# bgmanuel99/Super-Resolution-Images-for-3D-Printing-Defect-Detection

Measured on AMD Instinct MI355X. Metric: 4x-SR MPix/s on 512x512 LR batch, higher is better.
Workload: dtype bf16

## Files before the change

### super-resolution-images-for-3d-printing-defect-detection_amd/csrc/dense_fused.hip

```cpp
#include <stdlib.h>
#include <string.h>

#include <type_traits>

#include "conv_common.h"

namespace {

struct ChainParams {
    const char* in; int in_nch;
    char* out; int out_nch;
    const char* so; int so_nch;
    const char* w;
    const float* bias;
    const char* zero;
    int B, H;
    int rows_per_wg; unsigned magic;
    float alpha, xscale, oscale;
    int dbg_flags;
    unsigned long long* dbg;
};

__device__ __forceinline__ f32x4 mma16(bf16x8 a, bf16x8 b, f32x4 c) { return __builtin_amdgcn_mfma_f32_16x16x32_bf16(a, b, c, 0, 0, 0); }

constexpr int ROWB = 3072;
constexpr int NSTG = 11;
constexpr int STGB = NSTG * ROWB;
constexpr int WINR = 10;
constexpr int ZERO_PAGE_BYTES = sr_ctx::ZERO_PAGE_BYTES;

template <int NB0, int NB1, int MODE> struct ChainLds {
    static constexpr int WSLOT = (NB0 + NB1) * 3 * 1024;
    static constexpr int NSB = MODE == 0 ? 3 : 2;
    static constexpr int NWS = MODE == 0 ? 2 : 3;
    static constexpr int BYTES = NSB * STGB + WINR * ROWB + NWS * WSLOT + (NB0 + NB1) * 16 * 4;
};

typedef unsigned u32x2 __attribute__((ext_vector_type(2)));
typedef unsigned u32x4 __attribute__((ext_vector_type(4)));
#define CHAIN_STAMP(k) do { if (STAMP && blockIdx.x < 64 && G < 64 && (wave == 0 || wave == 5 || wave == 8 || wave == 11) && lane == 0)                \
        p.dbg[(((size_t)blockIdx.x * 4 + (wave == 0 ? 0 : wave == 5 ? 1 : wave == 8 ? 2 : 3)) * 64 + G) * 4 + (k)] = __builtin_amdgcn_s_memtime(); } while (0)

template <int N, class F> __device__ __forceinline__ void static_for(F&& f) {
    if constexpr (N > 0) {
        static_for<N - 1>(f);
        f(std::integral_constant<int, N - 1>{});
    }
}

template <int N> __device__ __forceinline__ void wait_imm() {
    static_assert(N >= 0 && N < 64, "vmcnt is a 6-bit counter");
    asm volatile("s_waitcnt vmcnt(%0)" ::"n"(N) : "memory");
}

template <int EXT, int NB0, int NB1, int MODE, int LW> struct LoaderPlan {
    static constexpr int NBT = NB0 + NB1, EXTG = 3 * EXT, NGR = 3 * (EXT + 1);
    static constexpr int RT_E = MODE == 1 ? 2 : 3;
    static constexpr int RT_R = 2;
    static constexpr int nrows(int kx) { return kx == 0 ? 2 : kx == 1 ? (LW < 3 ? 1 : 0) : 0; }
    static constexpr int nst_at(int i) {
        i = (i % NGR + NGR) % NGR;
        return i < EXTG ? 3 * nrows(i % 3) : 0;
    }
    static constexpr int nwdma(int iw) {
        const bool ext = iw < EXTG;
        const int nw = ext ? NBT * 3 : NB1 * 3, rt = ext ? RT_E : RT_R;
        int n = 0;
        for (int t = 0; t < (nw + 3) / 4; ++t)
            if (LW + 4 * t < nw && t >= rt) ++n;
        return n;
    }
};

constexpr bool kDirectStores = true;
constexpr int NCOMP = 8, NLOAD = 4;

template <int EXT, int NB0, int NB1, int MODE, bool HAS_O, bool STAMP, bool SEAM = false>
__global__ void __launch_bounds__((NCOMP + NLOAD) * 64, (NCOMP + NLOAD + 3) / 4) chain2_kernel(ChainParams p) {
    using L = ChainLds<NB0, NB1, MODE>;
    constexpr int NBT = NB0 + NB1, WSLOT = L::WSLOT;
    constexpr int NGR = 3 * (EXT + 1);
    constexpr int EXTG = 3 * EXT;
    constexpr int NTHR = (NCOMP + NLOAD) * 64;
    extern __shared__ __attribute__((aligned(16))) char smem[];
    char* const stg = smem;
    constexpr int NSB = L::NSB;
    char* const win = smem + NSB * STGB;
    char* const wr = win + WINR * ROWB;
    constexpr int NWS = L::NWS;
    float* const lbias = reinterpret_cast<float*>(wr + NWS * WSLOT);

    const int tid = threadIdx.x, lane = tid & 63, px = lane & 15, q = lane >> 4;
    const int wave = __builtin_amdgcn_readfirstlane(tid >> 6);
    const int H = p.H, Hp1 = H + 1;
    const int T = p.B * Hp1;
    const int R0 = blockIdx.x * p.rows_per_wg, R1 = min(T, R0 + p.rows_per_wg);
    if (R0 >= R1) return;
    const int Rs = R0 - 1;
    const int N = R1 - Rs + 1;
    const int nsteps = (N + 1 + 7) >> 3;

    for (int u = tid; u < WINR * ROWB / 16; u += NTHR) *reinterpret_cast<f32x4*>(win + u * 16) = f32x4{0.f, 0.f, 0.f, 0.f};
    if (tid < NBT * 16) lbias[tid] = p.bias[tid];
    asm volatile("s_waitcnt lgkmcnt(0)" ::: "memory");
    __builtin_amdgcn_s_barrier();

    auto row_of = [&](int g, int& img, int& y) -> bool {
        const int gg = Rs + g;
        if (gg < 0 || gg >= T) return false;
        img = (int)__umulhi((unsigned)gg, p.magic);
        y = gg - img * Hp1;
        return y < H;
    };
    auto own = [&](int g) { return Rs + g >= R0 && Rs + g < R1; };
    int G = 0;
    auto dma = [&](const char* src, char* dst) {
        __builtin_amdgcn_global_load_lds((const __attribute__((address_space(1))) void*)src, (__attribute__((address_space(3))) void*)dst, 16, 0, 0);
    };
    if (wave >= NCOMP) {
        const int lwr = wave - NCOMP;
        const int lsrc = 64 * (lane >> 2) + 16 * ((lane & 3) ^ (2 * ((lane >> 4) & 1)));
        auto loader = [&](auto LWc) {
            constexpr int LW = decltype(LWc)::value;
            auto row_base = [&](int s2, int j) -> const char* {
                int img, y;
                const bool real = row_of(8 * s2 - 2 + j, img, y);
                return real ? p.in + ((int64_t)img * H + y) * p.in_nch * ROWB : p.zero;
            };
            using Plan = LoaderPlan<EXT, NB0, NB1, MODE, LW>;
            const char* rb_cur[3];
            const char* rb_nxt[3];
            auto bases_of = [&](int s2, const char* (&rb)[3]) {
                rb[0] = row_base(s2, LW);
                rb[1] = row_base(s2, LW + 4);
                rb[2] = row_base(s2, 8 + (LW < 3 ? LW : 2));
            };
            auto stage_row = [&](auto Jc, const char* rb, int c1, char* sdst) {
                constexpr int j = decltype(Jc)::value;
                const char* src = rb + c1 * ROWB + lsrc;
                char* dst = sdst + j * ROWB;
                const auto gs = (const __attribute__((address_space(1))) void*)src;
                const auto ld = (__attribute__((address_space(3))) void*)dst;
                if constexpr (j < 8) {
                    __builtin_amdgcn_global_load_lds(gs, ld, 16, 0, 2);
                    __builtin_amdgcn_global_load_lds(gs, ld, 16, 1024, 2);
                    __builtin_amdgcn_global_load_lds(gs, ld, 16, 2048, 2);
                } else {
                    __builtin_amdgcn_global_load_lds(gs, ld, 16, 0, 0);
                    __builtin_amdgcn_global_load_lds(gs, ld, 16, 1024, 0);
                    __builtin_amdgcn_global_load_lds(gs, ld, 16, 2048, 0);
                }
            };
            auto stage_rows = [&](auto KXc, const char* (&rb)[3], int c1, char* sdst) {
                constexpr int kx = decltype(KXc)::value;
                if constexpr (kx == 0) {
                    stage_row(std::integral_constant<int, LW>{}, rb[0], c1, sdst);
                    stage_row(std::integral_constant<int, LW + 4>{}, rb[1], c1, sdst);
                } else if constexpr (kx == 1 && LW < 3) {
                    stage_row(std::integral_constant<int, 8 + (LW < 3 ? LW : 0)>{}, rb[2], c1, sdst);
                }
            };
            constexpr int RT_E = Plan::RT_E, RT_R = Plan::RT_R;
            u32x4 wre[EXTG][RT_E], wrr[3][RT_R];
            auto wsrc_of = [&](int iw) { return p.w + (iw < EXTG ? iw * WSLOT : EXTG * WSLOT + (iw - EXTG) * (NB1 * 3 * 1024)); };
#pragma unroll
            for (int iw = 0; iw < EXTG; ++iw)
#pragma unroll
                for (int t = 0; t < RT_E; ++t)
                    if (LW + 4 * t < NBT * 3) wre[iw][t] = *reinterpret_cast<const u32x4*>(wsrc_of(iw) + (LW + 4 * t) * 1024 + lane * 16);
#pragma unroll
            for (int r = 0; r < 3; ++r)
#pragma unroll
                for (int t = 0; t < RT_R; ++t)
                    if (LW + 4 * t < NB1 * 3) wrr[r][t] = *reinterpret_cast<const u32x4*>(wsrc_of(EXTG + r) + (LW + 4 * t) * 1024 + lane * 16);
            auto put_weights = [&](auto IW, int Gw) {
                constexpr int iw = decltype(IW)::value;
                constexpr bool ext = iw < EXTG;
                constexpr int nw = ext ? NBT * 3 : NB1 * 3, rt = ext ? RT_E : RT_R;
                const char* wq = p.w;
                asm volatile("" : "+s"(wq));
                const char* wsrc = wq + (ext ? iw * WSLOT : EXTG * WSLOT + (iw - EXTG) * (NB1 * 3 * 1024)) + lane * 16;
                char* wdst = wr + (Gw % NWS) * WSLOT;
#pragma unroll
                for (int t = 0; t < (nw + 3) / 4; ++t) {
                    const int k = LW + 4 * t;
                    if (k < nw) {
                        if (t < rt) {
                            if constexpr (ext) *reinterpret_cast<u32x4*>(wdst + k * 1024 + lane * 16) = wre[ext ? iw : 0][t < RT_E ? t : 0];
                            else *reinterpret_cast<u32x4*>(wdst + k * 1024 + lane * 16) = wrr[ext ? 0 : iw - EXTG][t < RT_R ? t : 0];
                        } else {
                            dma(wsrc + k * 1024, wdst + k * 1024);
                        }
                    }
                }
            };
            constexpr int WL = NWS - 1;
            constexpr int SL = NSB - 1;
            static_assert(MODE == 1 || (RT_E * NLOAD >= NBT * 3 && RT_R * NLOAD >= NB1 * 3), "growth pairs: every weight piece is resident (no weight DMA in the counted waits)");
            static_assert(SL <= EXT, "rows run at most one step ahead");
            static_for<WL>([&](auto I) { put_weights(I, decltype(I)::value); });
            bases_of(0, rb_cur);
            bases_of(1, rb_nxt);
            static_for<SL>([&](auto C0) {
                constexpr int c0 = decltype(C0)::value;
                stage_rows(std::integral_constant<int, 0>{}, rb_cur, c0, stg + c0 * STGB);
                stage_rows(std::integral_constant<int, 1>{}, rb_cur, c0, stg + c0 * STGB);
            });
            int nch = 0;
            for (int s = 0; s < nsteps; ++s) {
                static_for<NGR>([&](auto I) {
                    constexpr int i = decltype(I)::value;
                    CHAIN_STAMP(0);
                    if (G == 0) asm volatile("s_waitcnt vmcnt(0)" ::: "memory");
                    asm volatile("s_waitcnt lgkmcnt(0)" ::: "memory");
                    __builtin_amdgcn_s_barrier();
                    CHAIN_STAMP(1);
                    constexpr int i2 = (i + WL) % NGR;
                    put_weights(std::integral_constant<int, i2>{}, G + WL);
                    if constexpr (i < EXTG) {
                        constexpr int c = i / 3, kx = i - 3 * c;
                        constexpr int c1 = (c + SL) % EXT;
                        constexpr bool next_step = c + SL >= EXT;
                        char* sdst = stg + ((nch + SL) % NSB) * STGB;
                        stage_rows(std::integral_constant<int, kx>{}, next_step ? rb_nxt : rb_cur, c1, sdst);
                        if (kx == 2) ++nch;
                    }
                    CHAIN_STAMP(2);
                    if constexpr (MODE == 0) {
                        wait_imm<Plan::nst_at(i) + Plan::nst_at(i - 1) + Plan::nst_at(i - 2)>();
                    } else {
                        constexpr bool third = i < EXTG && i % 3 == 2;
                        wait_imm<Plan::nwdma(i2) + Plan::nst_at(i) + (third ? 0 : Plan::nst_at(i - 1))>();
                    }
                    CHAIN_STAMP(3);
                    ++G;
                });
                rb_cur[0] = rb_nxt[0]; rb_cur[1] = rb_nxt[1]; rb_cur[2] = rb_nxt[2];
                bases_of(s + 2, rb_nxt);
            }
            asm volatile("s_waitcnt vmcnt(0)" ::: "memory");
        };
        if (lwr == 0) loader(std::integral_constant<int, 0>{});
        else if (lwr == 1) loader(std::integral_constant<int, 1>{});
        else if (lwr == 2) loader(std::integral_constant<int, 2>{});
        else loader(std::integral_constant<int, 3>{});
        return;
    }

    int offk[3];
#pragma unroll
    for (int kx = 0; kx < 3; ++kx) {
        const int c = px + kx - 1;
        offk[kx] = 64 * c + 16 * (q ^ (2 * ((c >> 2) & 1)));
    }
    const bool edge_l = px == 0, edge_r = px == 15;
    const int off_l = edge_l ? offk[1] : offk[0];
    const int off_r = edge_r ? offk[1] : offk[2];
    const bool seam_l = SEAM && px == 8, seam_r = SEAM && px == 7;

    f32x4 a0[NB0][3], a1[NB1][3];

    auto transpose_offsets = [&](int& t_a, int& t_line) {
        int l = lane;
        asm volatile("" : "+v"(l));
        const int px_ = l & 15, q_ = l >> 4;
        t_a = px_ * 64 + 16 * ((q_ >> 1) ^ ((px_ >> 1) & 3)) + (q_ & 1) * 8;
        t_line = (l >> 2) * 64 + 16 * ((l & 3) ^ ((l >> 3) & 3));
    };

    auto xfold = [&](int h, float scale) {
        const bf16_t xs_b = (bf16_t)scale;
        int j0 = 16 * h + px - 8 * q;
        asm volatile("" : "+v"(j0));
        bf16x8 f;
#pragma unroll
        for (int j = 0; j < 8; ++j) f[j] = j == j0 ? xs_b : (bf16_t)0.f;
        return f;
    };
    constexpr int WDEPTH = 3, NWREG = WDEPTH + 1;
    struct ExtStage { int d, layer, n, frag, first; };
    auto ext_stage = [](int k) constexpr -> ExtStage {
        int i = 0;
        for (int d = 0; d < 4; ++d) {
            bool first = true;
            if (d >= 1)
                for (int n = 0; n < NB0; ++n, ++i, first = false)
                    if (i == k) return ExtStage{d, 0, n, (d - 1) * NB0 + n, first};
            if (d <= 2)
                for (int n = 0; n < NB1; ++n, ++i, first = false)
                    if (i == k) return ExtStage{d, 1, n, 3 * NB0 + d * NB1 + n, first};
        }
        return ExtStage{-1, 0, 0, 0, 0};
    };
    constexpr int NEXTST = 3 * (NB0 + NB1);
    auto ext_granule = [&](auto KXc, auto FOLDc, const char* sb, const char* ws) {
        constexpr int KX = decltype(KXc)::value;
        constexpr int FOLD = KX == 1 ? decltype(FOLDc)::value : -1;
        const char* rb = sb + wave * ROWB;
        auto load_row = [&](int d, bf16x8 (&x)[3]) {
#pragma unroll
            for (int cg = 0; cg < 3; ++cg) {
                const int off = (KX == 0 && cg == 0) ? off_l : (KX == 2 && cg == 2) ? off_r : offk[KX];
                x[cg] = *reinterpret_cast<const bf16x8*>(rb + d * ROWB + cg * 1024 + off);
                if ((KX == 0 && cg == 0 && edge_l) || (KX == 2 && cg == 2 && edge_r)) x[cg] = bf16x8{};
                if (SEAM && cg == 1 && ((KX == 0 && seam_l) || (KX == 2 && seam_r))) x[cg] = bf16x8{};
            }
        };
        auto ldw = [&](int frag) { return *reinterpret_cast<const bf16x8*>(ws + frag * 1024 + lane * 16); };
        bf16x8 xr[2][3], wq[NWREG];
        load_row(0, xr[0]);
        static_for<WDEPTH>([&](auto K) { wq[decltype(K)::value] = ldw(ext_stage(decltype(K)::value).frag); });
        static_for<NEXTST>([&](auto K) {
            constexpr int k = decltype(K)::value;
            constexpr ExtStage st = ext_stage(k);
            if constexpr (st.first && st.d < 3) load_row(st.d + 1, xr[(st.d + 1) & 1]);
            if constexpr (k + WDEPTH < NEXTST) wq[(k + WDEPTH) % NWREG] = ldw(ext_stage(k + WDEPTH).frag);
#pragma unroll
            for (int cg = 0; cg < 3; ++cg) {
                if constexpr (st.layer == 0) a0[st.n][cg] = mma16(wq[k % NWREG], xr[st.d & 1][cg], a0[st.n][cg]);
                else a1[st.n][cg] = mma16(wq[k % NWREG], xr[st.d & 1][cg], a1[st.n][cg]);
            }
            if constexpr (FOLD >= 0 && st.d == 1 && st.layer == 1 && st.n == NB1 - 1) {
#pragma unroll
                for (int h = 0; h < 2; ++h) {
                    const bf16x8 f = xfold(h, p.xscale);
#pragma unroll
                    for (int cg = 0; cg < 3; ++cg) a1[2 * FOLD + h][cg] = mma16(f, xr[1][cg], a1[2 * FOLD + h][cg]);
                }
            }
            __builtin_amdgcn_sched_barrier(0);
        });
    };
    constexpr int NRINGST = 3 * NB1;
    auto ring_granule = [&](auto KXc, int s, const char* ws) {
        constexpr int KX = decltype(KXc)::value;
        auto load_row = [&](int ky, bf16x8 (&x)[3]) {
            const char* rb = win + ((8 * s + wave - 2 + ky + 2 * WINR) % WINR) * ROWB;
#pragma unroll
            for (int cg = 0; cg < 3; ++cg) {
                const int off = (KX == 0 && cg == 0) ? off_l : (KX == 2 && cg == 2) ? off_r : offk[KX];
                x[cg] = *reinterpret_cast<const bf16x8*>(rb + cg * 1024 + off);
                if ((KX == 0 && cg == 0 && edge_l) || (KX == 2 && cg == 2 && edge_r)) x[cg] = bf16x8{};
                if (SEAM && cg == 1 && ((KX == 0 && seam_l) || (KX == 2 && seam_r))) x[cg] = bf16x8{};
            }
        };
        auto ldw = [&](int frag) { return *reinterpret_cast<const bf16x8*>(ws + frag * 1024 + lane * 16); };
        bf16x8 xr[2][3], wq[NWREG];
        load_row(0, xr[0]);
        static_for<WDEPTH>([&](auto K) { wq[decltype(K)::value] = ldw(decltype(K)::value); });
        static_for<NRINGST>([&](auto K) {
            constexpr int k = decltype(K)::value;
            constexpr int ky = k / NB1, n = k % NB1;
            if constexpr (n == 0 && ky < 2) load_row(ky + 1, xr[(ky + 1) & 1]);
            if constexpr (k + WDEPTH < NRINGST) wq[(k + WDEPTH) % NWREG] = ldw(k + WDEPTH);
#pragma unroll
            for (int cg = 0; cg < 3; ++cg) a1[n][cg] = mma16(wq[k % NWREG], xr[ky & 1][cg], a1[n][cg]);
            __builtin_amdgcn_sched_barrier(0);
        });
    };
    auto sync = [&]() {
        asm volatile("s_waitcnt lgkmcnt(0)" ::: "memory");
        __builtin_amdgcn_s_barrier();
    };

    int nch = 0;
    auto chunk = [&](auto FOLDc, int& Gr) {
        const char* sb = stg + (nch % NSB) * STGB;
#pragma unroll
        for (int kx = 0; kx < 3; ++kx, ++Gr) {
            CHAIN_STAMP(0);
            sync();
            CHAIN_STAMP(1);
            CHAIN_STAMP(2);
            const char* ws = wr + (Gr % NWS) * WSLOT;
            if (STAMP && (p.dbg_flags & 2)) {  }
            else if (kx == 0) ext_granule(std::integral_constant<int, 0>{}, FOLDc, sb, ws);
            else if (kx == 1) ext_granule(std::integral_constant<int, 1>{}, FOLDc, sb, ws);
            else ext_granule(std::integral_constant<int, 2>{}, FOLDc, sb, ws);
            CHAIN_STAMP(3);
        }
        ++nch;
    };
    for (int s = 0; s < nsteps; ++s) {
#pragma unroll
        for (int n = 0; n < NB0; ++n) {
            const f32x4 b = *reinterpret_cast<const f32x4*>(lbias + n * 16 + 4 * q);
#pragma unroll
            for (int cg = 0; cg < 3; ++cg) a0[n][cg] = b;
        }
#pragma unroll
        for (int n = 0; n < NB1; ++n) {
            const f32x4 b = *reinterpret_cast<const f32x4*>(lbias + (NB0 + n) * 16 + 4 * q);
#pragma unroll
            for (int cg = 0; cg < 3; ++cg) a1[n][cg] = b;
        }
        if constexpr (MODE == 1) {
            static_assert(MODE == 0 || EXT >= 2, "the tail's skip spans chunks 0 and 1");
            chunk(std::integral_constant<int, 0>{}, G);
            chunk(std::integral_constant<int, 1>{}, G);
#pragma nounroll
            for (int c = 2; c < EXT; ++c) chunk(std::integral_constant<int, -1>{}, G);
        } else {
#pragma nounroll
            for (int c = 0; c < EXT; ++c) chunk(std::integral_constant<int, -1>{}, G);
        }
        {
            const int g0 = 8 * s + wave;
            int img, y;
            const bool real = row_of(g0, img, y);
            char* wrow = win + (g0 % WINR) * ROWB;
            char* grow = real && own(g0) && MODE == 0 ? const_cast<char*>(p.in) + (((int64_t)img * H + y) * p.in_nch + EXT) * ROWB : nullptr;
#pragma unroll
            for (int cg = 0; cg < 3; ++cg) {
                f32x4 v[NB0];
                bf16x4 ob[NB0];
#pragma unroll
                for (int n = 0; n < NB0; ++n) {
#pragma unroll
                    for (int e = 0; e < 4; ++e) v[n][e] = real ? fmaxf(a0[n][cg][e], 0.f) : 0.f;
                    const bf16x4 o = {(bf16_t)v[n][0], (bf16_t)v[n][1], (bf16_t)v[n][2], (bf16_t)v[n][3]};
                    ob[n] = o;
                    const int slice = n * 2 + (q >> 1);
                    *reinterpret_cast<bf16x4*>(wrow + cg * 1024 + 64 * px + 16 * (slice ^ (2 * ((px >> 2) & 1))) + (q & 1) * 8) = o;
                }
                if constexpr (MODE == 0 && NB0 == 2 && kDirectStores) {
                    if (grow) {
                        const u32x2 au = __builtin_bit_cast(u32x2, ob[0]), cu = __builtin_bit_cast(u32x2, ob[NB0 - 1]);
                        const auto s0 = __builtin_amdgcn_permlane16_swap(au[0], cu[0], false, false);
                        const auto s1 = __builtin_amdgcn_permlane16_swap(au[1], cu[1], false, false);
                        const u32x4 ov = {(unsigned)s0[0], (unsigned)s1[0], (unsigned)s0[1], (unsigned)s1[1]};
                        __builtin_nontemporal_store(ov, reinterpret_cast<u32x4*>(grow + cg * 1024 + 64 * px + 2 * ((q & 1) * 16 + 4 * (q & ~1))));
                    }
                }
            }
            if (MODE == 0 && grow && !(NB0 == 2 && kDirectStores)) {
                static_assert(MODE == 1 || NB0 == 2, "growth convs have 32 output channels");
                asm volatile("" ::: "memory");
#pragma unroll
                for (int cg = 0; cg < 3; ++cg) {
                    const u32x4 v = *reinterpret_cast<const u32x4*>(wrow + cg * 1024 + (lane >> 2) * 64 + 16 * ((lane & 3) ^ (2 * ((lane >> 4) & 1))));
                    __builtin_nontemporal_store(v, reinterpret_cast<u32x4*>(grow + cg * 1024 + lane * 16));
                }
            }
        }
        char* const tb = stg + ((nch + NSB - 1) % NSB) * STGB + wave * 4096;
        const char* sob = nullptr;
        if (MODE == 1 && HAS_O) {
            int img, y;
            if (row_of(8 * s + wave - 1, img, y) && own(8 * s + wave - 1)) sob = p.so + ((int64_t)img * H + y) * p.so_nch * ROWB;
        }
        auto so_fetch = [&](int cg) {
            if (MODE == 1 && HAS_O && sob) {
                int l = lane;
                asm volatile("" : "+v"(l));
                const int ls = 64 * (l >> 2) + 16 * ((l & 3) ^ (2 * ((l >> 4) & 1)));
                dma(sob + cg * 1024 + ls, tb);
                dma(sob + ROWB + cg * 1024 + ls, tb + 1024);
            }
        };
#pragma unroll
        for (int kx = 0; kx < 3; ++kx, ++G) {
            CHAIN_STAMP(0);
            sync();
            CHAIN_STAMP(1);
            so_fetch(kx);
            CHAIN_STAMP(2);
            const char* ws = wr + (G % NWS) * WSLOT;
            if (kx == 0) ring_granule(std::integral_constant<int, 0>{}, s, ws);
            else if (kx == 1) ring_granule(std::integral_constant<int, 1>{}, s, ws);
            else ring_granule(std::integral_constant<int, 2>{}, s, ws);
            if (MODE == 1 && HAS_O && sob) {
                asm volatile("s_waitcnt vmcnt(0)" ::: "memory");
                int l = lane;
                asm volatile("" : "+v"(l));
                const int pxl = l & 15, ql = l >> 4;
                const int offc = 64 * pxl + 16 * (ql ^ (2 * ((pxl >> 2) & 1)));
#pragma unroll
                for (int c2 = 0; c2 < 2; ++c2) {
                    const bf16x8 xo = *reinterpret_cast<const bf16x8*>(tb + c2 * 1024 + offc);
#pragma unroll
                    for (int h = 0; h < 2; ++h) a1[2 * c2 + h][kx] = mma16(xfold(h, p.oscale), xo, a1[2 * c2 + h][kx]);
                }
            }
            CHAIN_STAMP(3);
        }
        {
            int img, y;
            const bool real = row_of(8 * s + wave - 1, img, y) && own(8 * s + wave - 1);
            if (real && !(STAMP && (p.dbg_flags & 1))) {
                const int64_t rowi = (int64_t)img * H + y;
                char* const grow = MODE == 0 ? const_cast<char*>(p.in) + (rowi * p.in_nch + EXT + 1) * ROWB : p.out + rowi * p.out_nch * ROWB;
                const float alpha = p.alpha;
                int t_a, t_line;
                transpose_offsets(t_a, t_line);
                if constexpr (MODE == 0 && NB1 == 2 && kDirectStores) {
#pragma unroll
                    for (int cg = 0; cg < 3; ++cg) {
                        bf16x4 ob[2];
#pragma unroll
                        for (int n = 0; n < 2; ++n)
                            ob[n] = bf16x4{(bf16_t)fmaxf(a1[n][cg][0], 0.f), (bf16_t)fmaxf(a1[n][cg][1], 0.f), (bf16_t)fmaxf(a1[n][cg][2], 0.f), (bf16_t)fmaxf(a1[n][cg][3], 0.f)};
                        const u32x2 au = __builtin_bit_cast(u32x2, ob[0]), cu = __builtin_bit_cast(u32x2, ob[1]);
                        const auto s0 = __builtin_amdgcn_permlane16_swap(au[0], cu[0], false, false);
                        const auto s1 = __builtin_amdgcn_permlane16_swap(au[1], cu[1], false, false);
                        const u32x4 ov = {(unsigned)s0[0], (unsigned)s1[0], (unsigned)s0[1], (unsigned)s1[1]};
                        __builtin_nontemporal_store(ov, reinterpret_cast<u32x4*>(grow + cg * 1024 + 64 * px + 2 * ((q & 1) * 16 + 4 * (q & ~1))));
                    }
                } else
#pragma unroll
                for (int cg = 0; cg < 3; ++cg)
#pragma unroll
                    for (int h = 0; h < NB1 / 2; ++h) {
                        char* const slot = tb + ((2 * cg + h) & 3) * 1024;
#pragma unroll
                        for (int u = 0; u < 2; ++u) {
                            const int n = 2 * h + u;
                            f32x4 v;
#pragma unroll
                            for (int e = 0; e < 4; ++e) v[e] = MODE == 0 ? fmaxf(a1[n][cg][e], 0.f) : alpha * a1[n][cg][e];
                            *reinterpret_cast<bf16x4*>(slot + (t_a ^ (32 * u))) = bf16x4{(bf16_t)v[0], (bf16_t)v[1], (bf16_t)v[2], (bf16_t)v[3]};
                        }
                        asm volatile("" ::: "memory");
                        const u32x4 line = *reinterpret_cast<const u32x4*>(slot + t_line);
                        __builtin_nontemporal_store(line, reinterpret_cast<u32x4*>(grow + h * ROWB + cg * 1024 + lane * 16));
                    }
            }
        }
    }
}

struct Conv1Params {
    const char* in; int in_nch;
    const char* w;
    const float* bias;
    const char* zero;
    int B, H;
    int rows_per_wg; unsigned magic;
};

constexpr int C1_NSTG = 10;
constexpr int C1_STGB = C1_NSTG * ROWB;
constexpr int C1_NSB = 4;
constexpr int C1_WBYTES = 2 * 9 * 2 * 1024;
constexpr int C1_LDS = C1_NSB * C1_STGB + C1_WBYTES + 32 * 4;
static_assert(C1_LDS <= 160 * 1024, "LDS budget");

template <bool SEAM>
__global__ void __launch_bounds__((NCOMP + NLOAD) * 64, (NCOMP + NLOAD + 3) / 4) conv1_stream_kernel(Conv1Params p) {
    extern __shared__ __attribute__((aligned(16))) char smem[];
    char* const stg = smem;
    char* const lw = smem + C1_NSB * C1_STGB;
    float* const lbias = reinterpret_cast<float*>(lw + C1_WBYTES);
    constexpr int NTHR = (NCOMP + NLOAD) * 64;
    const int tid = threadIdx.x, lane = tid & 63, px = lane & 15, q = lane >> 4;
    const int wave = __builtin_amdgcn_readfirstlane(tid >> 6);
    const int H = p.H, Hp1 = H + 1;
    const int T = p.B * Hp1;
    const int R0 = blockIdx.x * p.rows_per_wg, R1 = min(T, R0 + p.rows_per_wg);
    if (R0 >= R1) return;
    const int nsteps = (R1 - R0 + 7) >> 3;
    const int nchunks = 2 * nsteps;

    for (int u = tid; u < C1_WBYTES / 16; u += NTHR) *reinterpret_cast<f32x4*>(lw + u * 16) = *reinterpret_cast<const f32x4*>(p.w + u * 16);
    if (tid < 32) lbias[tid] = p.bias[tid];

    auto row_of = [&](int g, int& img, int& y) -> bool {
        const int gg = R0 + g;
        if (gg < 0 || gg >= T) return false;
        img = (int)__umulhi((unsigned)gg, p.magic);
        y = gg - img * Hp1;
        return y < H;
    };
    if (wave >= NCOMP) {
        const int lwr = wave - NCOMP;
        const int lsrc = 64 * (lane >> 2) + 16 * ((lane & 3) ^ (2 * ((lane >> 4) & 1)));
        auto loader = [&](auto LWc) {
            constexpr int LW = decltype(LWc)::value;
            constexpr int NROWS = LW < 2 ? 3 : 2, NP = 3 * NROWS;
            auto stage_unit = [&](int k) {
                const int s2 = k >> 1, c = k & 1;
                char* const sdst = stg + (k % C1_NSB) * C1_STGB;
                static_for<NROWS>([&](auto Jc) {
                    constexpr int j = decltype(Jc)::value == 0 ? LW : decltype(Jc)::value == 1 ? LW + 4 : 8 + LW;
                    int img, y;
                    const bool real = k < nchunks && row_of(8 * s2 - 1 + j, img, y);
                    const char* src = (real ? p.in + (((int64_t)img * H + y) * p.in_nch + c) * ROWB : p.zero) + lsrc;
                    const auto gs = (const __attribute__((address_space(1))) void*)src;
                    const auto ld = (__attribute__((address_space(3))) void*)(sdst + j * ROWB);
                    __builtin_amdgcn_global_load_lds(gs, ld, 16, 0, 0);
                    __builtin_amdgcn_global_load_lds(gs, ld, 16, 1024, 0);
                    __builtin_amdgcn_global_load_lds(gs, ld, 16, 2048, 0);
                });
            };
            stage_unit(0); stage_unit(1); stage_unit(2);
            for (int k = 0; k < nchunks; ++k) {
                if (k == 0) wait_imm<2 * NP>();
                __builtin_amdgcn_s_barrier();
                stage_unit(k + 3);
                wait_imm<2 * NP>();
            }
            asm volatile("s_waitcnt vmcnt(0)" ::: "memory");
        };
        asm volatile("s_waitcnt vmcnt(0) lgkmcnt(0)" ::: "memory");
        if (lwr == 0) loader(std::integral_constant<int, 0>{});
        else if (lwr == 1) loader(std::integral_constant<int, 1>{});
        else if (lwr == 2) loader(std::integral_constant<int, 2>{});
        else loader(std::integral_constant<int, 3>{});
        return;
    }
    asm volatile("s_waitcnt vmcnt(0) lgkmcnt(0)" ::: "memory");
    int offk[3];
#pragma unroll
    for (int kx = 0; kx < 3; ++kx) {
        const int c = px + kx - 1;
        offk[kx] = 64 * c + 16 * (q ^ (2 * ((c >> 2) & 1)));
    }
    const bool edge_l = px == 0, edge_r = px == 15;
    const int off_l = edge_l ? offk[1] : offk[0];
    const int off_r = edge_r ? offk[1] : offk[2];
    typedef unsigned u32x2c __attribute__((ext_vector_type(2)));
    for (int s = 0; s < nsteps; ++s) {
        f32x4 acc[2][3];
#pragma unroll
        for (int c = 0; c < 2; ++c) {
            const int k = 2 * s + c;
            asm volatile("s_waitcnt lgkmcnt(0)" ::: "memory");
            __builtin_amdgcn_s_barrier();
            if (c == 0) {
#pragma unroll
                for (int n = 0; n < 2; ++n) {
                    const f32x4 b = *reinterpret_cast<const f32x4*>(lbias + n * 16 + 4 * q);
#pragma unroll
                    for (int cg = 0; cg < 3; ++cg) acc[n][cg] = b;
                }
            }
            const char* const sb = stg + (k % C1_NSB) * C1_STGB + wave * ROWB;
#pragma unroll
            for (int kx = 0; kx < 3; ++kx) {
                bf16x8 wf[3][2];
#pragma unroll
                for (int ky = 0; ky < 3; ++ky)
#pragma unroll
                    for (int n = 0; n < 2; ++n) wf[ky][n] = *reinterpret_cast<const bf16x8*>(lw + (((c * 9) + ky * 3 + kx) * 2 + n) * 1024 + lane * 16);
#pragma unroll
                for (int ky = 0; ky < 3; ++ky) {
#pragma unroll
                    for (int cg = 0; cg < 3; ++cg) {
                        const int off = (kx == 0 && cg == 0) ? off_l : (kx == 2 && cg == 2) ? off_r : offk[kx];
                        bf16x8 x = *reinterpret_cast<const bf16x8*>(sb + ky * ROWB + cg * 1024 + off);
                        if ((kx == 0 && cg == 0 && edge_l) || (kx == 2 && cg == 2 && edge_r)) x = bf16x8{};
                        if (SEAM && cg == 1 && ((kx == 0 && px == 8) || (kx == 2 && px == 7))) x = bf16x8{};
#pragma unroll
                        for (int n = 0; n < 2; ++n) acc[n][cg] = mma16(wf[ky][n], x, acc[n][cg]);
                    }
                }
            }
        }
        int img, y;
        const int g = 8 * s + wave;
        if (g < R1 - R0 && row_of(g, img, y)) {
            char* const grow = const_cast<char*>(p.in) + (((int64_t)img * H + y) * p.in_nch + 2) * ROWB;
            const int lane_b = 64 * px + 2 * ((q & 1) * 16 + 4 * (q & ~1));
#pragma unroll
            for (int cg = 0; cg < 3; ++cg) {
                bf16x4 o[2];
#pragma unroll
                for (int n = 0; n < 2; ++n)
                    o[n] = bf16x4{(bf16_t)fmaxf(acc[n][cg][0], 0.f), (bf16_t)fmaxf(acc[n][cg][1], 0.f), (bf16_t)fmaxf(acc[n][cg][2], 0.f), (bf16_t)fmaxf(acc[n][cg][3], 0.f)};
                const u32x2c au = __builtin_bit_cast(u32x2c, o[0]), cu = __builtin_bit_cast(u32x2c, o[1]);
                const auto s0 = __builtin_amdgcn_permlane16_swap(au[0], cu[0], false, false);
                const auto s1 = __builtin_amdgcn_permlane16_swap(au[1], cu[1], false, false);
                const u32x4 ov = {(unsigned)s0[0], (unsigned)s1[0], (unsigned)s0[1], (unsigned)s1[1]};
                __builtin_nontemporal_store(ov, reinterpret_cast<u32x4*>(grow + cg * 1024 + lane_b));
            }
        }
    }
}

template <int EXT, int NB0, int NB1, int MODE>
int launch_chain(sr_ctx* ctx, const ChainParams& p, bool has_o, int nwg, bool seam, hipStream_t st) {
    constexpr int lds = ChainLds<NB0, NB1, MODE>::BYTES;
    static_assert(lds <= 160 * 1024, "LDS budget");
    if (seam) {
        if (has_o) {
            auto k = chain2_kernel<EXT, NB0, NB1, MODE, true, false, true>;
            if (int rc = ctx->ensure_dyn_lds(reinterpret_cast<const void*>(k), lds)) return rc;
            hipLaunchKernelGGL(k, dim3(nwg), dim3((NCOMP + NLOAD) * 64), lds, st, p);
        } else {
            auto k = chain2_kernel<EXT, NB0, NB1, MODE, false, false, true>;
            if (int rc = ctx->ensure_dyn_lds(reinterpret_cast<const void*>(k), lds)) return rc;
            hipLaunchKernelGGL(k, dim3(nwg), dim3((NCOMP + NLOAD) * 64), lds, st, p);
        }
    } else if (p.dbg) {
        auto k = chain2_kernel<EXT, NB0, NB1, MODE, MODE == 1, true>;
        if (int rc = ctx->ensure_dyn_lds(reinterpret_cast<const void*>(k), lds)) return rc;
        ChainParams q = p;
        if (MODE == 1 && !has_o) { q.so = p.in; q.so_nch = p.in_nch; q.oscale = 0.f; }
        hipLaunchKernelGGL(k, dim3(nwg), dim3((NCOMP + NLOAD) * 64), lds, st, q);
    } else if (has_o) {
        auto k = chain2_kernel<EXT, NB0, NB1, MODE, true, false>;
        if (int rc = ctx->ensure_dyn_lds(reinterpret_cast<const void*>(k), lds)) return rc;
        hipLaunchKernelGGL(k, dim3(nwg), dim3((NCOMP + NLOAD) * 64), lds, st, p);
    } else {
        auto k = chain2_kernel<EXT, NB0, NB1, MODE, false, false>;
        if (int rc = ctx->ensure_dyn_lds(reinterpret_cast<const void*>(k), lds)) return rc;
        hipLaunchKernelGGL(k, dim3(nwg), dim3((NCOMP + NLOAD) * 64), lds, st, p);
    }
    SR_HIP(ctx, hipGetLastError());
    return SR_OK;
}

}

int chain_pack_weights(sr_ctx* ctx, const float* wa, const float* ba, const float* wb, const float* bb, int ext, int nb0, int nb1, ChainWeights* out) {
    const int cin_a = 32 * ext, cin_b = 32 * (ext + 1), cout_a = 16 * nb0, cout_b = 16 * nb1;
    const size_t nfrag = (size_t)3 * ext * 3 * (nb0 + nb1) + (size_t)3 * 3 * nb1;
    std::vector<uint16_t> host(nfrag * 512);
    size_t idx = 0;
    auto frag = [&](const float* w, int cin, int cout, int c, int ky, int kx, int blk) {
        for (int l = 0; l < 64; ++l)
            for (int j = 0; j < 8; ++j)
                host[idx++] = f32_to_bf16_host(w[((size_t)(ky * 3 + kx) * cin + 32 * c + 8 * (l >> 4) + j) * cout + 16 * blk + (l & 15)]);
    };
    for (int c = 0; c < ext; ++c)
        for (int kx = 0; kx < 3; ++kx) {
            for (int ky = 0; ky < 3; ++ky) for (int n = 0; n < nb0; ++n) frag(wa, cin_a, cout_a, c, ky, kx, n);
            for (int ky = 0; ky < 3; ++ky) for (int n = 0; n < nb1; ++n) frag(wb, cin_b, cout_b, c, ky, kx, n);
        }
    for (int kx = 0; kx < 3; ++kx)
        for (int ky = 0; ky < 3; ++ky) for (int n = 0; n < nb1; ++n) frag(wb, cin_b, cout_b, ext, ky, kx, n);
    ChainWeights cw;
    cw.ext = ext; cw.nb0 = nb0; cw.nb1 = nb1;
    cw.bytes = host.size() * 2;
    std::vector<float> hb(cout_a + cout_b, 0.f);
    if (ba) for (int i = 0; i < cout_a; ++i) hb[i] = ba[i];
    if (bb) for (int i = 0; i < cout_b; ++i) hb[cout_a + i] = bb[i];
    if (int rc = weights_upload(ctx, host.data(), cw.bytes, hb.data(), (int)hb.size(), (int)hb.size(), &cw.w, &cw.bias)) return rc;
    *out = cw;
    return SR_OK;
}

bool conv1_stream_supported(const ConvWeights& w, const TensorView& in, int W) {
    return w.w != nullptr && w.rows && w.dtype == SR_DTYPE_BF16 && w.KS == 3 && w.Cin == 64 && w.Cout == 32 && w.NT == 2 && w.nchunks == 2 && W == 48 && in.blk &&
           in.coff == 0 && in.cs % 32 == 0 && in.cs >= 96;
}

int conv1_stream_launch(sr_ctx* ctx, const ConvWeights& w, TensorView in, int B, int H, int W, hipStream_t st, bool seam) {
    if (!conv1_stream_supported(w, in, W)) return ctx->fail(SR_ERR_INVALID, "streaming conv1: needs a 64 -> 32 bf16 3x3 conv on a 48-pixel-wide row-blocked buffer");
    if (B <= 0 || H <= 0) return ctx->fail(SR_ERR_INVALID, "streaming conv1: empty tensor");
    if (!ctx->zero_page) return ctx->fail(SR_ERR_STATE, "context has no zero page");
    int ncu = ctx->cu_count();
    if (ctx->chain_max_wgs > 0 && ctx->chain_max_wgs < ncu) ncu = ctx->chain_max_wgs;
    Conv1Params p;
    p.in = static_cast<const char*>(in.p); p.in_nch = (int)(in.cs / 32);
    p.w = static_cast<const char*>(w.w); p.bias = w.bias; p.zero = static_cast<const char*>(ctx->zero_page);
    p.B = B; p.H = H;
    const int64_t T = (int64_t)B * (H + 1);
    if ((T + 16) * (int64_t)(H + 1) * (H + 1) >= (1ll << 32)) return ctx->fail(SR_ERR_INVALID, "streaming conv1: stream too long");
    const int nwg_target = (int)std::max<int64_t>(1, std::min<int64_t>(ncu, (T + 15) / 16));
    p.rows_per_wg = (int)((T + nwg_target - 1) / nwg_target);
    const int nwg = (int)((T + p.rows_per_wg - 1) / p.rows_per_wg);
    p.magic = (unsigned)(((1ull << 32) + (unsigned)H) / (unsigned)(H + 1));
    int rec = -1;
    if (ctx->prof) {
        const double px = (double)B * H * W;
        rec = ctx->prof_open("dense_conv1_stream<bf16,64->32>", 2.0 * px * 9.0 * 64 * 32, px * 2.0 * (64 + 32), st);
    }
    auto k = seam ? conv1_stream_kernel<true> : conv1_stream_kernel<false>;
    if (int rc = ctx->ensure_dyn_lds(reinterpret_cast<const void*>(k), C1_LDS)) return rc;
    hipLaunchKernelGGL(k, dim3(nwg), dim3((NCOMP + NLOAD) * 64), C1_LDS, st, p);
    ctx->prof_close(rec, st);
    SR_HIP(ctx, hipGetLastError());
    return SR_OK;
}

bool chain_supported(const ChainWeights& w, const TensorView& in, int W) {
    return w.w != nullptr && W == 48 && in.blk && in.coff == 0 && in.cs % 32 == 0 && in.cs >= 32 * (w.ext + (w.nb1 == 4 ? 1 : 2));
}

int chain_launch(sr_ctx* ctx, const ChainWeights& w, TensorView in, int B, int H, int W, TensorView out, TensorView skip_o, float alpha,
                 float beta_x, float beta_o, hipStream_t st, bool seam) {
    if (!chain_supported(w, in, W)) return ctx->fail(SR_ERR_INVALID, "fused dense-block pair: needs W == 48 and a row-blocked source buffer");
    if (B <= 0 || H <= 0) return ctx->fail(SR_ERR_INVALID, "fused dense-block pair: empty tensor");
    const bool tail = w.nb1 == 4;
    if (tail && (!out.p || !out.blk || out.coff != 0 || out.cs % 32 != 0 || alpha == 0.f)) return ctx->fail(SR_ERR_INVALID, "fused dense-block tail: bad destination view");
    if (skip_o.p && (!skip_o.blk || skip_o.coff != 0 || skip_o.cs % 32 != 0)) return ctx->fail(SR_ERR_INVALID, "fused dense-block tail: bad skip view");
    static_assert(ZERO_PAGE_BYTES >= 6 * ROWB, "zero page covers every chunk offset");
    if (!ctx->zero_page) return ctx->fail(SR_ERR_STATE, "context has no zero page");
    int ncu = ctx->num_cus;
    if (ncu <= 0) {
        hipDeviceProp_t prop;
        SR_HIP(ctx, hipGetDeviceProperties(&prop, ctx->device));
        ncu = ctx->num_cus = prop.multiProcessorCount > 0 ? prop.multiProcessorCount : 256;
    }
    if (ctx->chain_max_wgs > 0 && ctx->chain_max_wgs < ncu) ncu = ctx->chain_max_wgs;
    ChainParams p;
    p.in = static_cast<const char*>(in.p); p.in_nch = (int)(in.cs / 32);
    p.out = static_cast<char*>(const_cast<void*>(out.p)); p.out_nch = (int)(out.cs / 32);
    p.so = static_cast<const char*>(skip_o.p); p.so_nch = (int)(skip_o.cs / 32);
    p.w = static_cast<const char*>(w.w); p.bias = w.bias; p.zero = static_cast<const char*>(ctx->zero_page);
    p.B = B; p.H = H;
    const int64_t T = (int64_t)B * (H + 1);
    if ((T + 16) * (int64_t)(H + 1) * (H + 1) >= (1ll << 32)) return ctx->fail(SR_ERR_INVALID, "fused dense-block pair: stream too long");
    const int nwg_target = (int)std::max<int64_t>(1, std::min<int64_t>(ncu, (T + 23) / 24));
    p.rows_per_wg = (int)((T + nwg_target - 1) / nwg_target);
    const int nwg = (int)((T + p.rows_per_wg - 1) / p.rows_per_wg);
    p.magic = (unsigned)(((1ull << 32) + (unsigned)H) / (unsigned)(H + 1));
    p.alpha = alpha; p.xscale = tail ? beta_x / alpha : 0.f; p.oscale = tail && skip_o.p ? beta_o / alpha : 0.f;
    for (float sc : {p.xscale, p.oscale}) {
        uint32_t u = (uint32_t)f32_to_bf16_host(sc) << 16;
        float back;
        memcpy(&back, &u, 4);
        if (back != sc) return ctx->fail(SR_ERR_INVALID, "fused dense-block tail: beta / alpha is not exactly representable in bf16");
    }
    p.dbg = ctx->chain_stamp_buf;
    { const char* f = getenv("SR355_CHAIN_DBG_FLAGS"); p.dbg_flags = f ? atoi(f) : 0; }
    if (p.dbg && ctx->chain_stamp_skip >= 0 && ctx->chain_stamp_skip-- != 0) p.dbg = nullptr;
    if (p.dbg && ctx->chain_stamp_skip == -1 && getenv("SR355_CHAIN_STAMP_SKIP")) ctx->chain_stamp_buf = nullptr;
    int rec = -1;
    if (ctx->prof) {
        const double px = (double)B * H * W;
        const double cin_a = 32.0 * w.ext, cin_b = 32.0 * (w.ext + 1), ca = 16.0 * w.nb0, cb = 16.0 * w.nb1;
        double bytes = px * 2.0 * (cin_a + (tail ? cb : ca + cb));
        if (tail && skip_o.p) bytes += px * 2.0 * 64.0;
        rec = ctx->prof_open(tail ? "dense_tail_fused<bf16,conv4+conv5>" : "dense_pair_fused<bf16>", 2.0 * px * 9.0 * (cin_a * ca + cin_b * cb), bytes, st);
    }
    int rc;
    const bool has_o = skip_o.p != nullptr;
    if (tail && w.ext == 5 && w.nb0 == 2) rc = launch_chain<5, 2, 4, 1>(ctx, p, has_o, nwg, seam, st);
    else if (!tail && w.ext == 2 && w.nb0 == 2 && w.nb1 == 2) rc = launch_chain<2, 2, 2, 0>(ctx, p, false, nwg, seam, st);
    else if (!tail && w.ext == 3 && w.nb0 == 2 && w.nb1 == 2) rc = launch_chain<3, 2, 2, 0>(ctx, p, false, nwg, seam, st);
    else rc = ctx->fail(SR_ERR_INVALID, "fused dense-block pair: shape not instantiated");
    ctx->prof_close(rec, st);
    return rc;
}
```

Baseline: 109.8.

## Carry weight and input prefetch across granule boundaries in chain kernel

Adds a carry plan so that, in MODE 1 without stamping, each granule prefetches the next granule's first weight fragments and first input row before its own MMA stream ends. The barrier then waits on only a partial lgkmcnt rather than draining all LDS loads. Weight packing is reordered so fragments are read sequentially in stage order. LDS address-space pointers and hoisted per-lane offsets cut address arithmetic. The risks are higher VGPR pressure from the wider weight queue, and correctness that depends on the partial waitcnt counts matching the prefetches actually issued.

After: 111.3, median of 6. +1.4%, better.

```diff
diff --git a/super-resolution-images-for-3d-printing-defect-detection_amd/csrc/dense_fused.hip b/super-resolution-images-for-3d-printing-defect-detection_amd/csrc/dense_fused.hip
--- a/super-resolution-images-for-3d-printing-defect-detection_amd/csrc/dense_fused.hip
+++ b/super-resolution-images-for-3d-printing-defect-detection_amd/csrc/dense_fused.hip
@@ -71,6 +71,14 @@
         return n;
     }
 };
+
+template <int EXT, int MODE, bool CARRY> struct CarryPlan {
+    static constexpr bool ext_w(int i) { return CARRY && i > 0 && i < 3 * EXT; }
+    static constexpr bool ext_x(int i) { return ext_w(i) && (i % 3 != 0 || MODE == 0); }
+    static constexpr bool ring_w(int kx) { return CARRY && kx > 0 && kx < 3; }
+    static constexpr bool ring_x(int kx) { return ring_w(kx); }
+};
+template <int MODE> constexpr bool kCarry = MODE == 1;
 
 constexpr bool kDirectStores = true;
 constexpr int NCOMP = 8, NLOAD = 4;
@@ -269,6 +277,7 @@
     };
 
     auto xfold = [&](int h, float scale) {
+        asm volatile("" : "+s"(scale));
         const bf16_t xs_b = (bf16_t)scale;
         int j0 = 16 * h + px - 8 * q;
         asm volatile("" : "+v"(j0));
@@ -277,48 +286,64 @@
         for (int j = 0; j < 8; ++j) f[j] = j == j0 ? xs_b : (bf16_t)0.f;
         return f;
     };
-    constexpr int WDEPTH = 3, NWREG = WDEPTH + 1;
-    struct ExtStage { int d, layer, n, frag, first; };
+    constexpr int WDEPTH = 3, NWQ = 6;
+    bf16x8 xr[2][3], wq[NWQ];
+    constexpr bool CARRY = kCarry<MODE> && !STAMP;
+    struct ExtStage { int d, layer, n, first; };
     auto ext_stage = [](int k) constexpr -> ExtStage {
         int i = 0;
         for (int d = 0; d < 4; ++d) {
             bool first = true;
             if (d >= 1)
                 for (int n = 0; n < NB0; ++n, ++i, first = false)
-                    if (i == k) return ExtStage{d, 0, n, (d - 1) * NB0 + n, first};
+                    if (i == k) return ExtStage{d, 0, n, first};
             if (d <= 2)
                 for (int n = 0; n < NB1; ++n, ++i, first = false)
-                    if (i == k) return ExtStage{d, 1, n, 3 * NB0 + d * NB1 + n, first};
-        }
-        return ExtStage{-1, 0, 0, 0, 0};
-    };
-    constexpr int NEXTST = 3 * (NB0 + NB1);
-    auto ext_granule = [&](auto KXc, auto FOLDc, const char* sb, const char* ws) {
+                    if (i == k) return ExtStage{d, 1, n, first};
+        }
+        return ExtStage{-1, 0, 0, 0};
+    };
+    constexpr int NEXTST = 3 * (NB0 + NB1), NRINGST = 3 * NB1;
+    static_assert(NEXTST % NWQ == 0 && NRINGST % NWQ == 0 && WDEPTH < NWQ, "a stage's wq entry must not depend on the granule in front of it");
+    auto load_row = [&](auto KXc, const char* row, bf16x8 (&x)[3]) {
         constexpr int KX = decltype(KXc)::value;
+#pragma unroll
+        for (int cg = 0; cg < 3; ++cg) {
+            const int off = (KX == 0 && cg == 0) ? off_l : (KX == 2 && cg == 2) ? off_r : offk[KX];
+            x[cg] = *reinterpret_cast<const bf16x8*>(row + cg * 1024 + off);
+            if ((KX == 0 && cg == 0 && edge_l) || (KX == 2 && cg == 2 && edge_r)) x[cg] = bf16x8{};
+            if (SEAM && cg == 1 && ((KX == 0 && seam_l) || (KX == 2 && seam_r))) x[cg] = bf16x8{};
+        }
+    };
+    typedef const __attribute__((address_space(3))) char* lds_cptr;
+    auto wlane = [&](const char* ws) {
+        lds_cptr wl = (lds_cptr)(ws + lane * 16);
+        asm volatile("" : "+v"(wl));
+        return wl;
+    };
+    auto ldw = [&](lds_cptr wl, int frag) { return *reinterpret_cast<const __attribute__((address_space(3))) bf16x8*>(wl + frag * 1024); };
+    auto ext_granule = [&](auto Ic, auto FOLDc, const char* sb, const char* sbn, const char* ws, const char* wsn) {
+        constexpr int I = decltype(Ic)::value, KX = I % 3;
         constexpr int FOLD = KX == 1 ? decltype(FOLDc)::value : -1;
+        using CP = CarryPlan<EXT, MODE, CARRY>;
+        constexpr bool IN_W = CP::ext_w(I), IN_X = CP::ext_x(I), OUT_W = CP::ext_w(I + 1) && I + 1 < EXTG, OUT_X = CP::ext_x(I + 1) && I + 1 < EXTG;
         const char* rb = sb + wave * ROWB;
-        auto load_row = [&](int d, bf16x8 (&x)[3]) {
-#pragma unroll
-            for (int cg = 0; cg < 3; ++cg) {
-                const int off = (KX == 0 && cg == 0) ? off_l : (KX == 2 && cg == 2) ? off_r : offk[KX];
-                x[cg] = *reinterpret_cast<const bf16x8*>(rb + d * ROWB + cg * 1024 + off);
-                if ((KX == 0 && cg == 0 && edge_l) || (KX == 2 && cg == 2 && edge_r)) x[cg] = bf16x8{};
-                if (SEAM && cg == 1 && ((KX == 0 && seam_l) || (KX == 2 && seam_r))) x[cg] = bf16x8{};
-            }
-        };
-        auto ldw = [&](int frag) { return *reinterpret_cast<const bf16x8*>(ws + frag * 1024 + lane * 16); };
-        bf16x8 xr[2][3], wq[NWREG];
-        load_row(0, xr[0]);
-        static_for<WDEPTH>([&](auto K) { wq[decltype(K)::value] = ldw(ext_stage(decltype(K)::value).frag); });
+        const lds_cptr wl = wlane(ws);
+        lds_cptr wln = nullptr;
+        if constexpr (!IN_X) load_row(std::integral_constant<int, KX>{}, rb, xr[0]);
+        if constexpr (!IN_W) static_for<WDEPTH>([&](auto K) { wq[decltype(K)::value] = ldw(wl, decltype(K)::value); });
         static_for<NEXTST>([&](auto K) {
             constexpr int k = decltype(K)::value;
             constexpr ExtStage st = ext_stage(k);
-            if constexpr (st.first && st.d < 3) load_row(st.d + 1, xr[(st.d + 1) & 1]);
-            if constexpr (k + WDEPTH < NEXTST) wq[(k + WDEPTH) % NWREG] = ldw(ext_stage(k + WDEPTH).frag);
+            if constexpr (st.first && st.d < 3) load_row(std::integral_constant<int, KX>{}, rb + (st.d + 1) * ROWB, xr[(st.d + 1) & 1]);
+            if constexpr (st.first && st.d == 3 && OUT_X) load_row(std::integral_constant<int, (KX + 1) % 3>{}, sbn + wave * ROWB, xr[0]);
+            if constexpr (k + WDEPTH == NEXTST && OUT_W) wln = wlane(wsn);
+            if constexpr (k + WDEPTH < NEXTST) wq[(k + WDEPTH) % NWQ] = ldw(wl, k + WDEPTH);
+            else if constexpr (OUT_W) wq[(k + WDEPTH) % NWQ] = ldw(wln, k + WDEPTH - NEXTST);
 #pragma unroll
             for (int cg = 0; cg < 3; ++cg) {
-                if constexpr (st.layer == 0) a0[st.n][cg] = mma16(wq[k % NWREG], xr[st.d & 1][cg], a0[st.n][cg]);
-                else a1[st.n][cg] = mma16(wq[k % NWREG], xr[st.d & 1][cg], a1[st.n][cg]);
+                if constexpr (st.layer == 0) a0[st.n][cg] = mma16(wq[k % NWQ], xr[st.d & 1][cg], a0[st.n][cg]);
+                else a1[st.n][cg] = mma16(wq[k % NWQ], xr[st.d & 1][cg], a1[st.n][cg]);
             }
             if constexpr (FOLD >= 0 && st.d == 1 && st.layer == 1 && st.n == NB1 - 1) {
 #pragma unroll
@@ -331,78 +356,78 @@
             __builtin_amdgcn_sched_barrier(0);
         });
     };
-    constexpr int NRINGST = 3 * NB1;
-    auto ring_granule = [&](auto KXc, int s, const char* ws) {
-        constexpr int KX = decltype(KXc)::value;
-        auto load_row = [&](int ky, bf16x8 (&x)[3]) {
-            const char* rb = win + ((8 * s + wave - 2 + ky + 2 * WINR) % WINR) * ROWB;
-#pragma unroll
-            for (int cg = 0; cg < 3; ++cg) {
-                const int off = (KX == 0 && cg == 0) ? off_l : (KX == 2 && cg == 2) ? off_r : offk[KX];
-                x[cg] = *reinterpret_cast<const bf16x8*>(rb + cg * 1024 + off);
-                if ((KX == 0 && cg == 0 && edge_l) || (KX == 2 && cg == 2 && edge_r)) x[cg] = bf16x8{};
-                if (SEAM && cg == 1 && ((KX == 0 && seam_l) || (KX == 2 && seam_r))) x[cg] = bf16x8{};
-            }
-        };
-        auto ldw = [&](int frag) { return *reinterpret_cast<const bf16x8*>(ws + frag * 1024 + lane * 16); };
-        bf16x8 xr[2][3], wq[NWREG];
-        load_row(0, xr[0]);
-        static_for<WDEPTH>([&](auto K) { wq[decltype(K)::value] = ldw(decltype(K)::value); });
+    auto ring_granule = [&](auto KXc, int s, const char* ws, const char* wsn) {
+        constexpr int KX = decltype(KXc)::value, XP = KX == 1 ? 1 : 0;
+        using CP = CarryPlan<EXT, MODE, CARRY>;
+        constexpr bool IN_W = CP::ring_w(KX), IN_X = CP::ring_x(KX), OUT_W = KX < 2 && CP::ring_w(KX + 1), OUT_X = KX < 2 && CP::ring_x(KX + 1);
+        auto rowp = [&](int ky) { return win + ((8 * s + wave - 2 + ky + 2 * WINR) % WINR) * ROWB; };
+        const lds_cptr wl = wlane(ws);
+        lds_cptr wln = nullptr;
+        if constexpr (!IN_X) load_row(KXc, rowp(0), xr[XP]);
+        if constexpr (!IN_W) static_for<WDEPTH>([&](auto K) { wq[decltype(K)::value] = ldw(wl, decltype(K)::value); });
         static_for<NRINGST>([&](auto K) {
             constexpr int k = decltype(K)::value;
             constexpr int ky = k / NB1, n = k % NB1;
-            if constexpr (n == 0 && ky < 2) load_row(ky + 1, xr[(ky + 1) & 1]);
-            if constexpr (k + WDEPTH < NRINGST) wq[(k + WDEPTH) % NWREG] = ldw(k + WDEPTH);
-#pragma unroll
-            for (int cg = 0; cg < 3; ++cg) a1[n][cg] = mma16(wq[k % NWREG], xr[ky & 1][cg], a1[n][cg]);
+            if constexpr (n == 0 && ky < 2) load_row(KXc, rowp(ky + 1), xr[(ky + 1 + XP) & 1]);
+            if constexpr (n == 0 && ky == 2 && OUT_X) load_row(std::integral_constant<int, (KX + 1) % 3>{}, rowp(0), xr[XP ^ 1]);
+            if constexpr (k + WDEPTH == NRINGST && OUT_W) wln = wlane(wsn);
+            if constexpr (k + WDEPTH < NRINGST) wq[(k + WDEPTH) % NWQ] = ldw(wl, k + WDEPTH);
+            else if constexpr (OUT_W) wq[(k + WDEPTH) % NWQ] = ldw(wln, k + WDEPTH - NRINGST);
+#pragma unroll
+            for (int cg = 0; cg < 3; ++cg) a1[n][cg] = mma16(wq[k % NWQ], xr[(ky + XP) & 1][cg], a1[n][cg]);
             __builtin_amdgcn_sched_barrier(0);
         });
     };
-    auto sync = [&]() {
-        asm volatile("s_waitcnt lgkmcnt(0)" ::: "memory");
+    auto sync = [&](auto NPREc) {
+        asm volatile("s_waitcnt lgkmcnt(%0)" ::"n"(decltype(NPREc)::value) : "memory");
         __builtin_amdgcn_s_barrier();
+        asm volatile("" ::: "memory");
     };
 
     int nch = 0;
-    auto chunk = [&](auto FOLDc, int& Gr) {
+    auto chunk = [&](auto Cc, auto FOLDc) {
+        constexpr int C = decltype(Cc)::value;
         const char* sb = stg + (nch % NSB) * STGB;
-#pragma unroll
-        for (int kx = 0; kx < 3; ++kx, ++Gr) {
+        const char* sbn = stg + ((nch + 1) % NSB) * STGB;
+        static_for<3>([&](auto KXc) {
+            constexpr int KX = decltype(KXc)::value, I = 3 * C + KX;
+            using CP = CarryPlan<EXT, MODE, CARRY>;
             CHAIN_STAMP(0);
-            sync();
+            sync(std::integral_constant<int, (CP::ext_w(I) ? WDEPTH : 0) + (CP::ext_x(I) ? 3 : 0)>{});
             CHAIN_STAMP(1);
             CHAIN_STAMP(2);
-            const char* ws = wr + (Gr % NWS) * WSLOT;
-            if (STAMP && (p.dbg_flags & 2)) {  }
-            else if (kx == 0) ext_granule(std::integral_constant<int, 0>{}, FOLDc, sb, ws);
-            else if (kx == 1) ext_granule(std::integral_constant<int, 1>{}, FOLDc, sb, ws);
-            else ext_granule(std::integral_constant<int, 2>{}, FOLDc, sb, ws);
+            ext_granule(std::integral_constant<int, I>{}, FOLDc, sb, KX == 2 ? sbn : sb, wr + (G % NWS) * WSLOT, wr + ((G + 1) % NWS) * WSLOT);
             CHAIN_STAMP(3);
-        }
+            ++G;
+        });
         ++nch;
     };
     for (int s = 0; s < nsteps; ++s) {
+        lds_cptr lb = (lds_cptr)(reinterpret_cast<const char*>(lbias) + 16 * q);
+        asm volatile("" : "+v"(lb));
 #pragma unroll
         for (int n = 0; n < NB0; ++n) {
-            const f32x4 b = *reinterpret_cast<const f32x4*>(lbias + n * 16 + 4 * q);
+            const f32x4 b = *reinterpret_cast<const __attribute__((address_space(3))) f32x4*>(lb + n * 64);
 #pragma unroll
             for (int cg = 0; cg < 3; ++cg) a0[n][cg] = b;
         }
 #pragma unroll
         for (int n = 0; n < NB1; ++n) {
-            const f32x4 b = *reinterpret_cast<const f32x4*>(lbias + (NB0 + n) * 16 + 4 * q);
+            const f32x4 b = *reinterpret_cast<const __attribute__((address_space(3))) f32x4*>(lb + (NB0 + n) * 64);
 #pragma unroll
             for (int cg = 0; cg < 3; ++cg) a1[n][cg] = b;
         }
-        if constexpr (MODE == 1) {
-            static_assert(MODE == 0 || EXT >= 2, "the tail's skip spans chunks 0 and 1");
-            chunk(std::integral_constant<int, 0>{}, G);
-            chunk(std::integral_constant<int, 1>{}, G);
+        static_assert(MODE == 0 || EXT >= 2, "the tail's skip spans chunks 0 and 1");
+        if constexpr (CARRY) {
+            static_for<EXT>([&](auto Cc) { chunk(Cc, std::integral_constant<int, (MODE == 1 && decltype(Cc)::value < 2) ? decltype(Cc)::value : -1>{}); });
+        } else if constexpr (MODE == 1) {
+            chunk(std::integral_constant<int, 0>{}, std::integral_constant<int, 0>{});
+            chunk(std::integral_constant<int, 1>{}, std::integral_constant<int, 1>{});
 #pragma nounroll
-            for (int c = 2; c < EXT; ++c) chunk(std::integral_constant<int, -1>{}, G);
+            for (int c = 2; c < EXT; ++c) chunk(std::integral_constant<int, 2>{}, std::integral_constant<int, -1>{});
         } else {
 #pragma nounroll
-            for (int c = 0; c < EXT; ++c) chunk(std::integral_constant<int, -1>{}, G);
+            for (int c = 0; c < EXT; ++c) chunk(std::integral_constant<int, 0>{}, std::integral_constant<int, -1>{});
         }
         {
             const int g0 = 8 * s + wave;
@@ -461,14 +486,16 @@
 #pragma unroll
         for (int kx = 0; kx < 3; ++kx, ++G) {
             CHAIN_STAMP(0);
-            sync();
+            if (kx == 0 || !CARRY) sync(std::integral_constant<int, 0>{});
+            else sync(std::integral_constant<int, WDEPTH + 3>{});
             CHAIN_STAMP(1);
             so_fetch(kx);
             CHAIN_STAMP(2);
             const char* ws = wr + (G % NWS) * WSLOT;
-            if (kx == 0) ring_granule(std::integral_constant<int, 0>{}, s, ws);
-            else if (kx == 1) ring_granule(std::integral_constant<int, 1>{}, s, ws);
-            else ring_granule(std::integral_constant<int, 2>{}, s, ws);
+            const char* wsn = wr + ((G + 1) % NWS) * WSLOT;
+            if (kx == 0) ring_granule(std::integral_constant<int, 0>{}, s, ws, wsn);
+            else if (kx == 1) ring_granule(std::integral_constant<int, 1>{}, s, ws, wsn);
+            else ring_granule(std::integral_constant<int, 2>{}, s, ws, wsn);
             if (MODE == 1 && HAS_O && sob) {
                 asm volatile("s_waitcnt vmcnt(0)" ::: "memory");
                 int l = lane;
@@ -493,6 +520,8 @@
                 const float alpha = p.alpha;
                 int t_a, t_line;
                 transpose_offsets(t_a, t_line);
+                int l16 = lane * 16;
+                asm volatile("" : "+v"(l16));
                 if constexpr (MODE == 0 && NB1 == 2 && kDirectStores) {
 #pragma unroll
                     for (int cg = 0; cg < 3; ++cg) {
@@ -522,7 +551,7 @@
                         }
                         asm volatile("" ::: "memory");
                         const u32x4 line = *reinterpret_cast<const u32x4*>(slot + t_line);
-                        __builtin_nontemporal_store(line, reinterpret_cast<u32x4*>(grow + h * ROWB + cg * 1024 + lane * 16));
+                        __builtin_nontemporal_store(line, reinterpret_cast<u32x4*>(grow + h * ROWB + cg * 1024 + l16));
                     }
             }
         }
@@ -723,10 +752,11 @@
                 host[idx++] = f32_to_bf16_host(w[((size_t)(ky * 3 + kx) * cin + 32 * c + 8 * (l >> 4) + j) * cout + 16 * blk + (l & 15)]);
     };
     for (int c = 0; c < ext; ++c)
-        for (int kx = 0; kx < 3; ++kx) {
-            for (int ky = 0; ky < 3; ++ky) for (int n = 0; n < nb0; ++n) frag(wa, cin_a, cout_a, c, ky, kx, n);
-            for (int ky = 0; ky < 3; ++ky) for (int n = 0; n < nb1; ++n) frag(wb, cin_b, cout_b, c, ky, kx, n);
-        }
+        for (int kx = 0; kx < 3; ++kx)
+            for (int d = 0; d < 4; ++d) {
+                if (d >= 1) for (int n = 0; n < nb0; ++n) frag(wa, cin_a, cout_a, c, d - 1, kx, n);
+                if (d <= 2) for (int n = 0; n < nb1; ++n) frag(wb, cin_b, cout_b, c, d, kx, n);
+            }
     for (int kx = 0; kx < 3; ++kx)
         for (int ky = 0; ky < 3; ++ky) for (int n = 0; n < nb1; ++n) frag(wb, cin_b, cout_b, ext, ky, kx, n);
     ChainWeights cw;
```
